# reunanen/annonet

Hardware: AMD Instinct MI355X
Metric: 227x227 RGB tiles/sec fwd+bwd @ batch 32 (higher is better)
Workload: dtype bf16; 1 GPU; training step (fwd+loss+bwd+SGD), batch 32x3x227x227 per GPU, encoder-decoder levels=2 width=1.0 K=3, random init; global_batch=32, parallelism=dp1

## Files before the change

annonet_amd/csrc/kernels_mfma.hip:

```cpp
#include <hip/hip_runtime.h>
#include <type_traits>

#include <algorithm>
#include <mutex>
#include <unordered_map>
#include <cstdio>
#include <vector>

#include "bnacc.h"
#include "common.h"
#include "kernels.h"

namespace anh {

void ensure_dynamic_lds(const void* kernel, size_t bytes) {
    if (bytes <= 64 * 1024) return;
    static std::mutex mu;
    static std::unordered_map<const void*, size_t> configured[64];
    int dev = 0;
    HIP_CHECK(hipGetDevice(&dev));
    std::lock_guard<std::mutex> lock(mu);
    size_t& have = configured[dev & 63][kernel];
    if (bytes > have) {
        HIP_CHECK(hipFuncSetAttribute(kernel, hipFuncAttributeMaxDynamicSharedMemorySize, (int)bytes));
// ... 845 lines not shown
        if constexpr (ONE_SET) {
            while (tile < total_tiles) {
                commit(ra, smem + (it & 1) * BUF_BYTES);
                if (tile + splits < total_tiles) fetch(ra, tile + splits);
                __syncthreads();
                tile += splits; ++it;
            }
        } else {
            if (tile + splits < total_tiles) fetch(rb, tile + splits);
            while (tile < total_tiles) {
                commit(ra, smem);
                if (tile + 2 * splits < total_tiles) fetch(ra, tile + 2 * splits);
                __syncthreads();
                tile += splits;
                if (tile >= total_tiles) break;
                commit(rb, smem + BUF_BYTES);
                if (tile + 2 * splits < total_tiles) fetch(rb, tile + 2 * splits);
                __syncthreads();
                tile += splits;
            }
        }
    } else {
        const int nt_mine = wave % NTC;
        int pofs[TPW][2], tofs[2];
#pragma unroll
        for (int i = 0; i < TPW; ++i) {
            const int j = wave + 4 * i, jc = j < 9 * NTC ? j : j - 4;
            const int tap = jc / NTC, ky = tap / 3, kx = tap - ky * 3;
            const int first = STRIDE == 1 ? ky * 34 + kx : (ky * 2 + (kx & 1)) * 33 + (kx >> 1);
            const int x_first = STRIDE == 1 ? kx : (kx >> 1);
#pragma unroll
            for (int rr = 0; rr < 2; ++rr) pofs[i][rr] = first * 64 + tr_lane_offset(lane, rr, x_first);
        }
#pragma unroll
        for (int rr = 0; rr < 2; ++rr) tofs[rr] = RECS * 64 + nt_mine * (TILE_PIX * 64) + tr_lane_offset(lane, rr, 0);
        f32x16 acc[TPW];
#pragma unroll
        for (int i = 0; i < TPW; ++i)
#pragma unroll
            for (int r = 0; r < 16; ++r) acc[i][r] = 0.f;
        for (; tile < total_tiles; tile += splits, ++it) {
            const char* lbuf = smem + (it & 1) * BUF_BYTES;
            const char* pa0[TPW];
            const char* pa1[TPW];
#pragma unroll
            for (int i = 0; i < TPW; ++i) { pa0[i] = lbuf + pofs[i][0]; pa1[i] = lbuf + pofs[i][1]; }
            const char* ta0 = lbuf + tofs[0];
            const char* ta1 = lbuf + tofs[1];
            __syncthreads();
            bf16x8 tf0, tf1, pf0[TPW], pf1[TPW];
            tf0 = tr_read8_at(ta0, ta1);
#pragma unroll
            for (int i = 0; i < TPW; ++i) pf0[i] = tr_read8_at(pa0[i], pa1[i]);
            wg_ksteps<0, KS, TPW, STRIDE, TRANS>(ta0, ta1, pa0, pa1, tf0, pf0, tf1, pf1, acc);
        }
        const size_t nw = (size_t)9 * a.c_in * a.c_out;
        float* out = a.partials + (size_t)split * nw;
        const int col = lane & 31, half = lane >> 5;
#pragma unroll
        for (int i = 0; i < TPW; ++i) {
            const int j = wave + 4 * i;
            if (j < 9 * NTC) {
                const int tap = j / NTC;
#pragma unroll
                for (int r = 0; r < 16; ++r) {
                    const int rowc = (r & 3) + 8 * (r >> 2) + 4 * half;
                    const int pch = cc + (TRANS ? col : rowc);
                    const int tch = tch0 + nt_mine * 32 + (TRANS ? rowc : col);
                    const int ci = TRANS ? tch : pch, co = TRANS ? pch : tch;
                    out[((size_t)tap * a.c_in + ci) * a.c_out + co] = acc[i][r];
                }
            }
        }
    }
}

__device__ __forceinline__ const char* swz_addr(const char* base, int rec, int key, int ks, int half) {
    return base + rec * 64 + ((((ks << 1) | half) ^ (key & 3)) << 4);
}
__device__ __forceinline__ bf16x8 lds_frag(const char* p) { return *reinterpret_cast<const bf16x8*>(p); }

struct GeoS1 {
    static constexpr int RECS = PATCH_PIX, ACC = 2;
    static constexpr bool RMW_PREFETCH = false;
    __device__ static void decode(int rec, int& py, int& px, int& key) { py = rec / PW; px = rec - py * PW; key = (px >> 2) & 3; }
    __device__ static int in_y0(int ty) { return ty * TH - 1; }
    __device__ static int in_x0(int tx) { return tx * TW - 1; }
    static constexpr int NB = 3;
    struct Bases { const char* x[3][2]; };
    __device__ static void init(Bases& b, const char* lds_x, int wave, int col, int half) {
#pragma unroll
        for (int kx = 0; kx < 3; ++kx)
#pragma unroll
            for (int ks = 0; ks < 2; ++ks) b.x[kx][ks] = swz_addr(lds_x, wave * 2 * PW + col + kx, (col + kx) >> 2, ks, half);
    }
    template <int NT>
    __device__ static void mfma(f32x16 (&acc)[ACC][NT], const Bases& b, const char* (&wb)[2]) {
        constexpr int C_OUT = NT * 32;
#pragma unroll
        for (int kx = 0; kx < 3; ++kx) {
#pragma unroll
            for (int ks = 0; ks < 2; ++ks) {
                bf16x8 xf[4];
#pragma unroll
                for (int r = 0; r < 4; ++r) xf[r] = lds_frag(b.x[kx][ks] + r * (PW * 64));
#pragma unroll
                for (int ky = 0; ky < 3; ++ky) {
                    const int tl = ky * 3 + kx;
#pragma unroll
                    for (int nt = 0; nt < NT; ++nt) {
                        const bf16x8 wf = lds_frag(wb[ks] + (tl * C_OUT + nt * 32) * 64);
#pragma unroll
                        for (int g = 0; g < 2; ++g) acc[g][nt] = __builtin_amdgcn_mfma_f32_32x32x16_bf16(wf, xf[g + ky], acc[g][nt], 0, 0, 0);
                    }
                }
            }
        }
    }
    __device__ static void load_filter_regs(bf16x8 (&wreg)[18], const char* (&wb)[2]) {
#pragma unroll
        for (int tl = 0; tl < 9; ++tl)
#pragma unroll
            for (int ks = 0; ks < 2; ++ks) wreg[tl * 2 + ks] = lds_frag(wb[ks] + (tl * 32) * 64);
    }
    __device__ static void mfma_wreg(f32x16 (&acc)[ACC][1], const Bases& b, const bf16x8 (&wreg)[18]) {
#pragma unroll
        for (int kx = 0; kx < 3; ++kx) {
#pragma unroll
            for (int ks = 0; ks < 2; ++ks) {
                bf16x8 xf[4];
#pragma unroll
                for (int r = 0; r < 4; ++r) xf[r] = lds_frag(b.x[kx][ks] + r * (PW * 64));
#pragma unroll
                for (int ky = 0; ky < 3; ++ky)
#pragma unroll
                    for (int g = 0; g < 2; ++g) acc[g][0] = __builtin_amdgcn_mfma_f32_32x32x16_bf16(wreg[(ky * 3 + kx) * 2 + ks], xf[g + ky], acc[g][0], 0, 0, 0);
            }
        }
    }
    __device__ static void out_pixel(int g, const ConvArgs& a, int n, int ty, int tx, int wave, int col, size_t& pix, bool& valid) {
        const int oy = ty * TH + wave * 2 + g, ox = tx * TW + col;
        valid = oy < a.h_out && ox < a.w_out;
        pix = ((size_t)n * a.h_out + (valid ? oy : 0)) * a.w_out + (valid ? ox : 0);
    }
};

struct GeoDown {
    static constexpr int RECS = 9 * 66, ACC = 1;
    static constexpr bool RMW_PREFETCH = false;
    __device__ static void decode(int rec, int& py, int& px, int& key) {
        py = rec / 66;
        const int rem = rec - py * 66, par = rem >= 33, u = rem - 33 * par;
        px = 2 * u + par; key = (u >> 2) & 3;
    }
    __device__ static int in_y0(int ty) { return ty * 8; }
    __device__ static int in_x0(int tx) { return tx * 64; }
    static constexpr int NB = 2;
    struct Bases { const char* x[2][2]; };
    __device__ static void init(Bases& b, const char* lds_x, int wave, int col, int half) {
#pragma unroll
        for (int kh = 0; kh < 2; ++kh)
#pragma unroll
            for (int ks = 0; ks < 2; ++ks) b.x[kh][ks] = swz_addr(lds_x, wave * 4 * 33 + col + kh, (col + kh) >> 2, ks, half);
    }
    template <int NT>
    __device__ static void mfma(f32x16 (&acc)[ACC][NT], const Bases& b, const char* (&wb)[2]) {
        constexpr int C_OUT = NT * 32;
#pragma unroll
        for (int tl = 0; tl < 9; ++tl) {
            const int ky = tl / 3, kx = tl - ky * 3;
#pragma unroll
            for (int ks = 0; ks < 2; ++ks) {
                const bf16x8 xf = lds_frag(b.x[kx >> 1][ks] + (ky * 2 + (kx & 1)) * (33 * 64));
#pragma unroll
                for (int nt = 0; nt < NT; ++nt) {
                    const bf16x8 wf = lds_frag(wb[ks] + (tl * C_OUT + nt * 32) * 64);
                    acc[0][nt] = __builtin_amdgcn_mfma_f32_32x32x16_bf16(wf, xf, acc[0][nt], 0, 0, 0);
                }
            }
        }
    }
    __device__ static void out_pixel(int, const ConvArgs& a, int n, int ty, int tx, int wave, int col, size_t& pix, bool& valid) {
        const int oy = ty * 4 + wave, ox = tx * 32 + col;
        valid = oy < a.h_out && ox < a.w_out;
        pix = ((size_t)n * a.h_out + (valid ? oy : 0)) * a.w_out + (valid ? ox : 0);
    }
};

struct GeoUp {
    static constexpr int RECS = 5 * 33, ACC = 4;
    static constexpr bool RMW_PREFETCH = true;
    __device__ static void decode(int rec, int& py, int& px, int& key) { py = rec / 33; px = rec - py * 33; key = (px >> 2) & 3; }
    __device__ static int in_y0(int ty) { return ty * 4 - 1; }
    __device__ static int in_x0(int tx) { return tx * 32 - 1; }
    static constexpr int NB = 2;
    struct Bases { const char* x[2][2]; };
    __device__ static void init(Bases& b, const char* lds_x, int wave, int col, int half) {
#pragma unroll
        for (int ib = 0; ib < 2; ++ib)
#pragma unroll
            for (int ks = 0; ks < 2; ++ks) b.x[ib][ks] = swz_addr(lds_x, wave * 33 + col + 1 - ib, (col + 1 - ib) >> 2, ks, half);
    }
    template <int NT>
    __device__ static void mfma(f32x16 (&acc)[ACC][NT], const Bases& b, const char* (&wb)[2]) {
        constexpr int C_OUT = NT * 32;
#pragma unroll
        for (int ks = 0; ks < 2; ++ks) {
            bf16x8 xf[2][2];
#pragma unroll
            for (int ia = 0; ia < 2; ++ia)
#pragma unroll
                for (int ib = 0; ib < 2; ++ib) xf[ia][ib] = lds_frag(b.x[ib][ks] + (1 - ia) * (33 * 64));
#pragma unroll
            for (int py = 0; py < 2; ++py)
#pragma unroll
                for (int px = 0; px < 2; ++px)
#pragma unroll
                    for (int ia = 0; ia < 2 - py; ++ia)
#pragma unroll
                        for (int ib = 0; ib < 2 - px; ++ib) {
                            const int tap = (py + 2 * ia) * 3 + px + 2 * ib;
#pragma unroll
                            for (int nt = 0; nt < NT; ++nt) {
                                const bf16x8 wf = lds_frag(wb[ks] + (tap * C_OUT + nt * 32) * 64);
                                acc[py * 2 + px][nt] = __builtin_amdgcn_mfma_f32_32x32x16_bf16(wf, xf[ia][ib], acc[py * 2 + px][nt], 0, 0, 0);
                            }
                        }
        }
    }
    __device__ static void out_pixel(int g, const ConvArgs& a, int n, int ty, int tx, int wave, int col, size_t& pix, bool& valid) {
        const int oy = 2 * (ty * 4 + wave) + (g >> 1), ox = 2 * (tx * 32 + col) + (g & 1);
        valid = oy < a.h_out && ox < a.w_out;
        pix = ((size_t)n * a.h_out + (valid ? oy : 0)) * a.w_out + (valid ? ox : 0);
    }
};

template <class G, int NT, int KIND, bool FWD = false, bool ACT = false, int PS = 0, bool HEAD = false>
__global__ __launch_bounds__(512, 2) void conv3x3_ws_kernel(ConvArgs a, int tiles_x, int tiles_y, int flip, long long* prof, int wres_, int e_off) {
#ifdef ANH_WS_PROFILE
    long long t_a = 0, t_b = 0, t_c = 0, t_d = 0, t0_;
    float prof_sink = 0.f;
    const bool prof_nostore = (wres_ >> 6) & 1;
    const long long t_entry = wall_clock64();
    long long t_loop = 0, t_loop_end = 0, c_loop = 0;
#define TICK() (t0_ = wall_clock64())
#define TOCK(acc_) (acc_ += wall_clock64() - t0_)
#else
#define TICK()
#define TOCK(acc_)
#endif
    static_assert(PS == 0 || PS == 1 || PS == 4 || PS == 5, "conv3x3_ws: producer-side forms 1 (sums), 4 (stores), 5 (both)");
    constexpr int NTHR = 512;
    constexpr int C_OUT = NT * 32, NP = (G::RECS * 4 + 255) / 256, W_ITEMS = 9 * C_OUT * 4, NW = (W_ITEMS + 255) / 256;
    constexpr int X_BYTES_ = G::RECS * 64, W_BYTES = 9 * C_OUT * 64, BUF = X_BYTES_ + W_BYTES;
    const int wres = wres_ & 1, bands = (wres_ >> 4) & 1;
    extern __shared__ __attribute__((aligned(16))) char smem[];
    const int n_slabs_l = a.c_red >> 5;
    const int x_stride = wres ? X_BYTES_ : BUF;
    const int w_base = 2 * X_BYTES_;
    const int tab_off = wres ? w_base + n_slabs_l * W_BYTES : 2 * BUF;
    float* tab = reinterpret_cast<float*>(smem + tab_off);

    const int hw_wave = __builtin_amdgcn_readfirstlane((int)threadIdx.x >> 6);
    const bool producer = hw_wave >= 4;
    const int wave = hw_wave & 3;
    const int lane = threadIdx.x & 63, tid = wave * 64 + lane, c16 = tid & 3;
    const int half = lane >> 5, col = lane & 31;
    const int co_base = blockIdx.y * C_OUT;
    const int H = a.h_in, W = a.w_in, c_red = a.c_red;
    const int n_slabs = c_red >> 5, n_tiles_all = tiles_x * tiles_y * a.n;
    const int band_len = (n_tiles_all + 7) >> 3;
    const int tile_first = bands ? (int)(blockIdx.x & 7) * band_len + (int)(blockIdx.x >> 3) : (int)blockIdx.x;
    const int gstep = bands ? (int)(gridDim.x >> 3) : (int)gridDim.x;
    const int n_tiles = bands ? min(n_tiles_all, ((int)(blockIdx.x & 7) + 1) * band_len) : n_tiles_all;
    constexpr bool CAN_STATS = G::ACC * NT <= 4 || FWD;
    const bool fuse_stats = !PS && !ACT && CAN_STATS && (a.stat_partials != nullptr || a.stat_acc != nullptr);
    const bool fuse_bnred = !FWD && (PS || CAN_STATS) && (a.bnred_partials != nullptr || a.bnred_acc != nullptr);
    constexpr bool PST = PS == 4 || PS == 5;
    const int stat_mode = fuse_stats ? 1 : (fuse_bnred && PS != 1 && PS != 5) ? 2 : 0;
    const bool ps = (PS == 1 || PS == 5) && fuse_bnred;
    const bool pst = PST && fuse_bnred;
    constexpr int E_BYTES = G::ACC * 128 * 64 * NT;
    constexpr int EK = 4 * NT, EQ_STEP = 256 / EK, ECH = G::ACC * 128 / EQ_STEP;
    float est[16];
    float* bnc = tab + c_red * 4;

    int tile = tile_first, slab = 0, it = 0;
    auto init_tables = [&]() __attribute__((always_inline)) {
        if (KIND == SRC_ACT || KIND == SRC_ACT2) {
            if (a.src.a_tab.acc) {
                const int sides = KIND == SRC_ACT2 ? 2 : 1;
                for (int i = threadIdx.x; i < sides * c_red; i += NTHR) {
                    const int side = i >= c_red, ch = i - side * c_red;
                    const BnTable& t = side ? a.src.b_tab : a.src.a_tab;
                    const BnFolded f = bnacc_fold_forward(t.acc, t.c, ch, t.pixels, t.gamma[ch], t.beta[ch], t.eps);
                    tab[2 * side * c_red + ch] = f.scale;
                    tab[(2 * side + 1) * c_red + ch] = f.shift;
                }
                if (KIND != SRC_ACT2) for (int i = threadIdx.x; i < c_red; i += NTHR) { tab[2 * c_red + i] = 0.f; tab[3 * c_red + i] = 0.f; }
            } else {
                for (int i = threadIdx.x; i < c_red; i += NTHR) {
                    tab[i] = a.src.a_scale[i];
                    tab[c_red + i] = a.src.a_shift[i];
                    tab[2 * c_red + i] = KIND == SRC_ACT2 ? a.src.b_scale[i] : 0.f;
                    tab[3 * c_red + i] = KIND == SRC_ACT2 ? a.src.b_shift[i] : 0.f;
                }
            }
        }
        if (ACT) {
            for (int i = threadIdx.x; i < C_OUT; i += NTHR) {
                bnc[i] = a.out_scale[co_base + i];
                bnc[C_OUT + i] = a.out_shift[co_base + i];
            }
        }
        if (fuse_bnred) {
            for (int i = threadIdx.x; i < C_OUT; i += NTHR) {
                bnc[i] = a.bnred_scale[co_base + i];
                bnc[C_OUT + i] = a.bnred_shift[co_base + i];
                bnc[2 * C_OUT + i] = a.bnred_mean[co_base + i];
                bnc[3 * C_OUT + i] = a.bnred_invstd[co_base + i];
            }
        }
        __syncthreads();
    };
    if (producer) {
        const bf16* wsrc = reinterpret_cast<const bf16*>(a.w_bf16);
        const bf16* xa = reinterpret_cast<const bf16*>(a.src.a);
        const bf16* xb = reinterpret_cast<const bf16*>(a.src.b);
        const size_t plane = (size_t)H * W * c_red;
        int pgeo[NP], pdst[NP];
    #pragma unroll
        for (int jj = 0; jj < NP; ++jj) {
            const int rec = min((tid >> 2) + 64 * jj, G::RECS - 1);
            int py, px, key;
            G::decode(rec, py, px, key);
            pgeo[jj] = py | (px << 8);
            pdst[jj] = rec * 64 + ((c16 ^ key) << 4);
        }
        int wsrc_off[NW], wdst[NW];
    #pragma unroll
        for (int j = 0; j < NW; ++j) {
            const int rec = min((tid >> 2) + 64 * j, 9 * C_OUT - 1);
            const int tl = rec / C_OUT, co = rec - tl * C_OUT;
            const int tap = flip ? 8 - tl : tl;
            wsrc_off[j] = (tap * a.c_out + co_base + co) * c_red + c16 * 8;
            wdst[j] = rec * 64 + ((c16 ^ ((co >> 2) & 3)) << 4);
        }
        u32x4 wraw[NW];
        struct Fetched {
            RawChunk<KIND> praw[NP];
            unsigned pok;
        };
        Fetched R0;
        const int per_img = tiles_x * tiles_y;
        const int step_x = gstep % tiles_x, step_y = (gstep / tiles_x) % tiles_y, step_n = gstep / per_img;
        int ftile = tile_first, fslab = 0;
        int ftx = ftile % tiles_x, fty = (ftile / tiles_x) % tiles_y, fn = ftile / per_img;
        constexpr bool NEED_MASK = KIND == SRC_ACT || KIND == SRC_ACT2;
        const int plane_bytes = (int)(unsigned)(plane * 2);
        int foff[NP];
        unsigned fpok = 0;
        auto enter_tile = [&]() __attribute__((always_inline)) {
            const int x0 = G::in_x0(ftx), y0 = G::in_y0(fty);
            fpok = 0;
    #pragma unroll
            for (int jj = 0; jj < NP; ++jj) {
                const int iy = y0 + (pgeo[jj] & 255), ix = x0 + (pgeo[jj] >> 8);
                const bool ok = (unsigned)iy < (unsigned)H && (unsigned)ix < (unsigned)W;
                foff[jj] = ok ? ((iy * W + ix) * c_red + c16 * 8) * 2 : (int)0xFFFFF000u;
                if constexpr (NEED_MASK) fpok |= (ok ? 1u : 0u) << jj;
            }
        };
        auto fetch = [&](Fetched& R) __attribute__((always_inline)) {
            const bf16* pa = xa + (size_t)fn * plane;
            const bf16* pb = (KIND == SRC_ACT2 || KIND == SRC_SUM2) ? xb + (size_t)fn * plane : nullptr;
            const int cc = fslab * 32;
            R.pok = fpok;
            const __amdgpu_buffer_rsrc_t ra = __builtin_amdgcn_make_buffer_rsrc(const_cast<bf16*>(pa), 0, plane_bytes, 0x00020000);
    #pragma unroll
            for (int jj = 0; jj < NP; ++jj) {
                const u32x4 v = __builtin_amdgcn_raw_buffer_load_b128(ra, foff[jj], cc * 2, 0);
                R.praw[jj].a = make_uint4(v[0], v[1], v[2], v[3]);
            }
            if constexpr (KIND == SRC_ACT2 || KIND == SRC_SUM2) {
                const __amdgpu_buffer_rsrc_t rb = __builtin_amdgcn_make_buffer_rsrc(const_cast<bf16*>(pb), 0, plane_bytes, 0x00020000);
    #pragma unroll
                for (int jj = 0; jj < NP; ++jj) {
                    const u32x4 v = __builtin_amdgcn_raw_buffer_load_b128(rb, foff[jj], cc * 2, 0);
                    R.praw[jj].b = make_uint4(v[0], v[1], v[2], v[3]);
                }
            }
            if (++fslab == n_slabs) {
                fslab = 0; ftile += gstep;
                ftx += step_x; if (ftx >= tiles_x) { ftx -= tiles_x; ++fty; }
                fty += step_y; if (fty >= tiles_y) { fty -= tiles_y; ++fn; }
                fn += step_n;
                if (ftile < n_tiles) enter_tile();
            }
        };
        const __amdgpu_buffer_rsrc_t rw = __builtin_amdgcn_make_buffer_rsrc(const_cast<bf16*>(wsrc), 0, 9 * a.c_out * c_red * 2, 0x00020000);
        auto fetch_w = [&](int slab_) __attribute__((always_inline)) {
    #pragma unroll
            for (int j = 0; j < NW; ++j) wraw[j] = __builtin_amdgcn_raw_buffer_load_b128(rw, wsrc_off[j] * 2, slab_ * 64, 0);
        };
        auto commit = [&](Fetched& R) __attribute__((always_inline)) {
            char* lbuf = smem + (it & 1) * x_stride;
            char* wbuf = lbuf + X_BYTES_;
            const bool stage_w = !wres && (it < 2 || n_slabs > 1);
            float sa[8], ta[8], sb[8], tb[8];
            if (KIND == SRC_ACT || KIND == SRC_ACT2) {
                const float* t0 = tab + slab * 32 + c16 * 8;
    #pragma unroll
                for (int j = 0; j < 8; ++j) {
                    sa[j] = t0[j]; ta[j] = t0[c_red + j];
                    sb[j] = KIND == SRC_ACT2 ? t0[2 * c_red + j] : 0.f;
                    tb[j] = KIND == SRC_ACT2 ? t0[3 * c_red + j] : 0.f;
                }
            }
    #pragma unroll
            for (int jj = 0; jj < NP; ++jj) {
                uint4 v = chunk_convert<KIND>(R.praw[jj], sa, ta, sb, tb);
                if constexpr (NEED_MASK) { if (!((R.pok >> jj) & 1u)) v = make_uint4(0u, 0u, 0u, 0u); }
                if ((tid >> 2) + 64 * jj < G::RECS) *reinterpret_cast<uint4*>(lbuf + pdst[jj]) = v;
            }
            if (stage_w) {
    #pragma unroll
                for (int j = 0; j < NW; ++j)
                    if ((tid >> 2) + 64 * j < 9 * C_OUT) *reinterpret_cast<u32x4*>(wbuf + wdst[j]) = wraw[j];
            }
        };
        if (ftile < n_tiles) { enter_tile(); fetch(R0); if (!wres) fetch_w(0); }
        if (wres && tile < n_tiles) {
            for (int sl = 0; sl < n_slabs; ++sl) {
                fetch_w(sl);
#pragma unroll
                for (int j = 0; j < NW; ++j)
                    if ((tid >> 2) + 64 * j < 9 * C_OUT) *reinterpret_cast<u32x4*>(smem + w_base + sl * W_BYTES + wdst[j]) = wraw[j];
            }
        }
        init_tables();
        float esc[8], esh[8];
        const int ek = tid & (EK - 1), eq0 = tid / EK;
        int hist1 = -1, hist2 = -1, hist1_it = 0, hist2_it = 0;
        if (PS == 1 || PS == 5) {
#pragma unroll
            for (int j = 0; j < 8; ++j) {
                esc[j] = bnc[ek * 8 + j]; esh[j] = bnc[C_OUT + ek * 8 + j];
                est[j] = 0.f; est[8 + j] = 0.f;
            }
        }
        const bf16* ylayer = reinterpret_cast<const bf16*>(a.bnred_y);
        unsigned epix[PST ? ECH : 1];
        auto estat_begin = [&](int et, u32x4 (&yv)[ECH], unsigned& evalid) __attribute__((always_inline)) {
            const int tx = et % tiles_x, ty = (et / tiles_x) % tiles_y, n = et / per_img;
            evalid = 0;
#pragma unroll
            for (int j = 0; j < ECH; ++j) {
                const int q = eq0 + EQ_STEP * j;
                size_t pix; bool valid;
                G::out_pixel(q >> 7, a, n, ty, tx, (q >> 5) & 3, q & 31, pix, valid);
                if (PS != 4) yv[j] = *reinterpret_cast<const u32x4*>(ylayer + pix * a.c_out + co_base + ek * 8);
                if constexpr (PST) epix[j] = (unsigned)pix;
                evalid |= (valid ? 1u : 0u) << j;
            }
        };
        auto estat_end = [&](int eit, const u32x4 (&yv)[ECH], unsigned evalid) __attribute__((always_inline)) {
            const char* eb = smem + e_off + (n_slabs == 1 ? (eit & 1) * E_BYTES : 0);
#pragma unroll
            for (int j = 0; j < ECH; ++j) {
                const int q = eq0 + EQ_STEP * j;
                const u32x4 dv = *reinterpret_cast<const u32x4*>(eb + q * (64 * NT) + ((ek ^ ebuf_swizzle<NT>(q)) << 4));
                if constexpr (PST) {
                    if ((evalid >> j) & 1u) store16(reinterpret_cast<bf16*>(a.out) + (size_t)epix[j] * a.c_out + co_base + ek * 8, make_uint4(dv[0], dv[1], dv[2], dv[3]));
                }
                if (PS != 4 && ((evalid >> j) & 1u)) {
#pragma unroll
                    for (int i = 0; i < 4; ++i)
#pragma unroll
                        for (int h2 = 0; h2 < 2; ++h2) {
                            const int c = 2 * i + h2;
                            const float d = h2 ? hi_f(dv[i]) : lo_f(dv[i]), y = h2 ? hi_f(yv[j][i]) : lo_f(yv[j][i]);
                            const float dz = fmaf(y, esc[c], esh[c]) > 0.f ? d : 0.f;
                            est[c] = fmaf(dz, y, est[c]);
                            est[8 + c] += dz;
                        }
                }
            }
        };
        auto one_item = [&](Fetched& R) __attribute__((always_inline)) {
            u32x4 eyv[PS ? ECH : 1];
            unsigned evalid = 0;
            const int et = hist2, eit = hist2_it;
            if constexpr (PS != 0) { if ((ps || pst) && et >= 0) estat_begin(et, eyv, evalid); }
            TICK();
            commit(R);
#ifdef ANH_WS_PROFILE
            __builtin_amdgcn_s_waitcnt(0xc07f);
#endif
            TOCK(t_a);
            TICK();
            if (ftile < n_tiles) fetch(R);
            if (!wres && n_slabs > 1 && (slab + 1 < n_slabs || tile + gstep < n_tiles)) fetch_w(slab + 1 < n_slabs ? slab + 1 : 0);
            if constexpr (PS != 0) { if ((ps || pst) && et >= 0) estat_end(eit, eyv, evalid); }
            TOCK(t_b);
            TICK();
            __syncthreads();
            TOCK(t_c);
            hist2 = hist1; hist2_it = hist1_it;
            hist1 = slab == n_slabs - 1 ? tile : -1; hist1_it = it;
            if (++slab == n_slabs) { slab = 0; tile += gstep; }
            ++it;
        };
#ifdef ANH_WS_PROFILE
        t_loop = wall_clock64();
        c_loop = clock64();
#endif
        while (tile < n_tiles) one_item(R0);
#ifdef ANH_WS_PROFILE
        t_loop_end = wall_clock64();
        c_loop = clock64() - c_loop;
#endif
        if constexpr (PS != 0) {
            if (ps || pst) {
                u32x4 eyv[ECH];
                unsigned evalid = 0;
                if (hist2 >= 0) { estat_begin(hist2, eyv, evalid); estat_end(hist2_it, eyv, evalid); }
                __syncthreads();
                if (hist1 >= 0) { estat_begin(hist1, eyv, evalid); estat_end(hist1_it, eyv, evalid); }
            }
        }
    } else {
        init_tables();
        typename G::Bases b0;
        G::init(b0, smem, wave, col, half);
        const char* wb0[2];
#pragma unroll
        for (int ks = 0; ks < 2; ++ks) wb0[ks] = swz_addr(smem, col, col >> 2, ks, half);
        f32x16 acc[G::ACC][NT];
        bf16x8 hw[2];
        float hbias[4] = {0.f, 0.f, 0.f, 0.f};
        if constexpr (HEAD) {
#pragma unroll
            for (int k = 0; k < 4; ++k) hbias[k] = k < a.head_k ? a.head_bias[k] : 0.f;
            head_operand(hw, a, col, half);
        }
        u32x4 old[FWD ? 1 : G::ACC][NT][2];
        u32x4 yraw[FWD ? 1 : G::ACC][NT][2];
        constexpr bool DEEP = !FWD && NT == 1 && G::RMW_PREFETCH;
        u32x4 old_n[DEEP ? G::ACC : 1][NT][2];
        const bool rmw_any = !FWD && G::RMW_PREFETCH && a.out_accumulate;
        const bool cons_bnred = fuse_bnred && PS != 1 && PS != 5;
        const bool pre_any = rmw_any || cons_bnred;
        auto prefetch_epilogue = [&](int t, auto& o, auto& y, bool want_old, bool want_y) __attribute__((always_inline)) {
            const int tx = t % tiles_x, ty = (t / tiles_x) % tiles_y, n = t / (tiles_x * tiles_y);
            const bf16* out = reinterpret_cast<const bf16*>(a.out);
            const bf16* yl = reinterpret_cast<const bf16*>(a.bnred_y);
#pragma unroll
            for (int g = 0; g < G::ACC; ++g) {
                size_t pix; bool valid;
                G::out_pixel(g, a, n, ty, tx, wave, col, pix, valid);
                const size_t e0 = pix * a.c_out + co_base + 8 * half;
#pragma unroll
                for (int nt = 0; nt < NT; ++nt)
#pragma unroll
                    for (int s2 = 0; s2 < 2; ++s2) {
                        if constexpr (!FWD) {
                            if (want_old) o[g][nt][s2] = *reinterpret_cast<const u32x4*>(out + e0 + nt * 32 + 16 * s2);
                            if (want_y) y[g][nt][s2] = *reinterpret_cast<const u32x4*>(yl + e0 + nt * 32 + 16 * s2);
                        }
                    }
            }
        };
        if (DEEP && pre_any && tile < n_tiles) prefetch_epilogue(tile, old, yraw, rmw_any, false);
        float stat[NT][2][16];
#pragma unroll
        for (int nt = 0; nt < NT; ++nt)
#pragma unroll
            for (int s2 = 0; s2 < 2; ++s2)
#pragma unroll
                for (int e = 0; e < 16; ++e) stat[nt][s2][e] = 0.f;
        constexpr bool WREG = std::is_same<G, GeoS1>::value && NT == 1;
        const bool wreg_on = WREG && n_slabs == 1 && !((wres_ >> 19) & 1);
        bf16x8 wreg[WREG ? 18 : 1];
        for (;;) {
            auto epilogue = [&](int et, int eit) __attribute__((always_inline)) {
                const int tx = et % tiles_x, ty = (et / tiles_x) % tiles_y, n = et / (tiles_x * tiles_y);
                const bool rmw = rmw_any;
#pragma unroll
                for (int g = 0; g < G::ACC; ++g) {
                    size_t pix; bool valid;
                    G::out_pixel(g, a, n, ty, tx, wave, col, pix, valid);
#ifdef ANH_WS_PROFILE
                    if (prof_nostore) valid = false;
#endif
                    if constexpr (HEAD) store_pixel_tiles_head(acc[g][0], a, pix, n, valid, half, bnc, C_OUT, hw, hbias);
                    else if constexpr (ACT) store_pixel_tiles_act<NT>(acc[g], a, pix, valid, half, co_base, bnc, C_OUT);
                    else {
                        const bool to_ebuf = ps || pst;
                        store_pixel_tiles_rmw<NT>(acc[g], a, pix, valid, half, co_base, old[FWD ? 0 : g], rmw, stat, stat_mode, yraw[FWD ? 0 : g], bnc,
                                                  to_ebuf ? smem + e_off + (n_slabs == 1 ? (eit & 1) * E_BYTES : 0) : nullptr, (g * 4 + wave) * 32 + col, !pst);
                    }
                }
                if constexpr (DEEP) {
                    if (pre_any) {
#pragma unroll
                        for (int g = 0; g < G::ACC; ++g)
#pragma unroll
                            for (int s2 = 0; s2 < 2; ++s2) old[g][0][s2] = old_n[g][0][s2];
                    }
                }
            };
            if (tile >= n_tiles) break;
            int ntile = tile, nslab = slab + 1;
            if (nslab == n_slabs) { nslab = 0; ntile += gstep; }
            const int boff = (it & 1) * x_stride;
            const int woff = wres ? w_base + slab * W_BYTES : boff + X_BYTES_;
            typename G::Bases b;
#pragma unroll
            for (int i = 0; i < G::NB; ++i)
#pragma unroll
                for (int ks = 0; ks < 2; ++ks) b.x[i][ks] = b0.x[i][ks] + boff;
            const char* wb[2] = {wb0[0] + woff, wb0[1] + woff};
            if (slab == 0) {
#pragma unroll
                for (int g = 0; g < G::ACC; ++g)
#pragma unroll
                    for (int nt = 0; nt < NT; ++nt)
#pragma unroll
                        for (int r = 0; r < 16; ++r) acc[g][nt][r] = 0.f;
            }
            TICK();
            __syncthreads();
            TOCK(t_c);
            TICK();
            const bool last_slab = slab == n_slabs - 1;
            if (pre_any && last_slab) {
                if constexpr (DEEP) {
                    if (tile + gstep < n_tiles) prefetch_epilogue(tile + gstep, old_n, yraw, rmw_any, false);
                    prefetch_epilogue(tile, old, yraw, false, cons_bnred);
                } else prefetch_epilogue(tile, old, yraw, rmw_any, cons_bnred);
            }
            if constexpr (WREG) {
                if (wreg_on) {
                    if (it == 0) G::load_filter_regs(wreg, wb);
                    G::mfma_wreg(acc, b, wreg);
                } else G::template mfma<NT>(acc, b, wb);
            } else G::template mfma<NT>(acc, b, wb);
#ifdef ANH_WS_PROFILE
            __builtin_amdgcn_sched_barrier(0);
#endif
            TOCK(t_a);
#ifdef ANH_WS_PROFILE
            TICK();
            if (last_slab) { asm volatile("v_mov_b32 %0, %1" : "=v"(prof_sink) : "v"(acc[0][0][0])); asm volatile("v_mov_b32 %0, %1" : "=v"(prof_sink) : "v"(acc[G::ACC - 1][NT - 1][15])); }
            __builtin_amdgcn_sched_barrier(0);
            TOCK(t_d);
#endif
            TICK();
            if (last_slab) epilogue(tile, it);
            TOCK(t_b);
            tile = ntile; slab = nslab; ++it;
        }
        if constexpr (PS != 0) { if (ps || pst) __syncthreads(); }
        if (stat_mode) {
            __syncthreads();
            float* red = reinterpret_cast<float*>(smem) + (size_t)(wave * 64 + lane) * (32 * NT);
#pragma unroll
            for (int nt = 0; nt < NT; ++nt)
#pragma unroll
// ... 27 lines not shown
            double* dst = fuse_stats ? a.stat_partials : a.bnred_partials;
            if (table) bnacc_add(table, (fuse_stats ? BNACC_SUM_Y : BNACC_SUM_DZ_XHAT) + which, a.c_out, co_base + ch, sum);
            else dst[((size_t)(co_base + ch) * 2 + which) * gridDim.x + blockIdx.x] = sum;
        }
    }
    if constexpr (PS == 1 || PS == 5) {
        if (ps) {
            __syncthreads();
            if (producer) {
                float* redw = reinterpret_cast<float*>(smem) + (size_t)tid * 16;
#pragma unroll
                for (int e = 0; e < 16; ++e) redw[e] = est[e];
            }
            __syncthreads();
            constexpr int GRP = 512 / (64 * NT);
            const int t = threadIdx.x / GRP, part = threadIdx.x % GRP;
            const int ch = t >> 1, which = t & 1, k = ch >> 3, j = ch & 7;
            const float* red = reinterpret_cast<const float*>(smem);
            double sum = 0.0;
#pragma unroll 4
            for (int m = part; m < EQ_STEP; m += GRP) sum += (double)red[(size_t)(k + EK * m) * 16 + which * 8 + j];
#pragma unroll
            for (int off = 1; off < GRP; off <<= 1) sum += __shfl_xor(sum, off, 64);
            {
                const double sum_dz = __shfl_down(sum, GRP, 64);
                if (which == 0) sum = (double)bnc[3 * C_OUT + ch] * (sum - (double)bnc[2 * C_OUT + ch] * sum_dz);
            }
            if (part == 0) {
                if (a.bnred_acc) bnacc_add(a.bnred_acc, BNACC_SUM_DZ_XHAT + which, a.c_out, co_base + ch, sum);
                else a.bnred_partials[((size_t)(co_base + ch) * 2 + which) * gridDim.x + blockIdx.x] = sum;
            }
        }
    }
    if (fuse_bnred && a.bnred_acc) bnacc_finish_backward(a.bnred_finish, (int)(gridDim.x * gridDim.y));
#ifdef ANH_WS_PROFILE
    if (prof && lane == 0) {
        long long* o = prof + ((size_t)(blockIdx.y * gridDim.x + blockIdx.x) * 8 + (producer ? 4 : 0) + wave) * 8;
        o[0] = t_a; o[1] = t_b; o[2] = t_c; o[3] = producer ? c_loop : it; o[4] = t_entry; o[5] = producer ? t_loop : t_d + (prof_sink == 12345.f ? 1 : 0); o[6] = t_loop_end; o[7] = wall_clock64();
    }
#endif
#undef TICK
#undef TOCK
}

int ws_target_wgs();

struct WsLayout { int wres; size_t lds; int ps ; int e_off; };
WsLayout ws_layout(const ConvArgs& a, int recs, int acc, int nt, bool with_bnred) {
    const size_t tables = (size_t)a.c_red * 16 + (size_t)nt * 32 * 16;
    const size_t x_bytes = (size_t)recs * 64, w_bytes = (size_t)9 * nt * 32 * 64;
    static const bool resident_on = !(getenv("ANH_WS_WEIGHT_RESIDENT") && atoi(getenv("ANH_WS_WEIGHT_RESIDENT")) == 0);
    const int n_slabs = a.c_red >> 5;
    const size_t resident_lds = 2 * x_bytes + (size_t)n_slabs * w_bytes + tables;
    WsLayout L{};
    L.wres = resident_on && n_slabs >= 2 && resident_lds <= 160 * 1024 && 2 * x_bytes + (size_t)n_slabs * w_bytes >= (size_t)32 * 1024 * nt;
    L.lds = L.wres ? resident_lds : 2 * (x_bytes + w_bytes) + tables;
    static const int ps_env = getenv("ANH_WS_PSTAT") ? atoi(getenv("ANH_WS_PSTAT")) : 7;
    int mode = 0;
    if (ps_env == 1) mode = acc == 4 ? 1 : 0;
    else if (ps_env == 8) mode = acc == 4 ? 1 : (acc * nt <= 4 ? 4 : 0);
    else mode = acc == 4 ? (nt == 1 ? 5 : 1) : (acc * nt <= 4 ? 4 : 0);
    const size_t e_total = (size_t)acc * 128 * 64 * nt * (n_slabs == 1 ? 2 : 1);
    if (mode && with_bnred && a.src.kind == SRC_RAW && !a.out_scale && !a.stat_partials && !a.stat_acc) {
        if (L.lds + e_total <= 160 * 1024) L.ps = mode;
        else if (n_slabs == 1 && resident_lds + e_total <= 160 * 1024 && resident_lds - tables >= 16 * 1024) { L.wres = 1; L.lds = resident_lds; L.ps = mode; }
    }
    L.e_off = L.ps ? (int)((L.lds + 15) / 16 * 16) : 0;
    if (L.ps) L.lds = (size_t)L.e_off + e_total;
    return L;
}

template <class G, int NT>
void launch_ws(const ConvArgs& a, int tiles_x, int tiles_y, int flip, hipStream_t s) {
    const int n_tiles = tiles_x * tiles_y * a.n, groups = a.c_out / (NT * 32);
    const dim3 grid((unsigned)std::max(1, std::min(n_tiles, ws_target_wgs() / groups)), (unsigned)groups);
    const WsLayout lay = ws_layout(a, G::RECS, G::ACC, NT, a.bnred_partials != nullptr || a.bnred_acc != nullptr);
    const int wres = lay.wres;
    const size_t lds = lay.lds;
    const int e_off = lay.e_off;
    static const int filter_regs_env = getenv("ANH_WS_FILTER_REGS") ? atoi(getenv("ANH_WS_FILTER_REGS")) : 1;
    const int ps = lay.ps;
    static const int bands_env = getenv("ANH_WS_XCD_BANDS") ? atoi(getenv("ANH_WS_XCD_BANDS")) : 1;
    const int bands = bands_env && grid.x % 8 == 0 && grid.x >= 8 ? 1 : 0;
    const int flags = wres | (bands << 4) | ((filter_regs_env ? 0 : 1) << 19);
    auto launch = [&](auto kernel) {
        const dim3 block(512);
        ensure_dynamic_lds(reinterpret_cast<const void*>(kernel), lds);
#ifndef ANH_WS_PROFILE
        hipLaunchKernelGGL(kernel, grid, block, lds, s, a, tiles_x, tiles_y, flip, (long long*)nullptr, flags, e_off);
#else
        static const int prof_on = getenv("ANH_WS_PROF") ? atoi(getenv("ANH_WS_PROF")) : 0;
        static long long* prof = nullptr;
        if (prof_on && !prof) HIP_CHECK(hipMalloc(&prof, 1024 * 12 * 8 * sizeof(long long)));
        static const int nostore = getenv("ANH_WS_PROF_NOSTORE") ? atoi(getenv("ANH_WS_PROF_NOSTORE")) : 0;
        hipLaunchKernelGGL(kernel, grid, block, lds, s, a, tiles_x, tiles_y, flip, prof_on ? prof : nullptr, flags | (nostore << 6), e_off);
        if (prof_on) {
            HIP_CHECK(hipStreamSynchronize(s));
            const int nwg = grid.x * grid.y, nw = 8, nc = 4;
            std::vector<long long> h((size_t)nwg * nw * 8);
            HIP_CHECK(hipMemcpy(h.data(), prof, h.size() * sizeof(long long), hipMemcpyDeviceToHost));
            double pa = 0, pb = 0, pc = 0, ca = 0, cb = 0, cc = 0, cd = 0, items = 0;
            long long first_entry = h[4], last_exit = h[7];
            double entry = 0, pro = 0, loop = 0, tail = 0, cycles = 0;
            for (int w = 0; w < nwg; ++w) {
                for (int v = 0; v < nw; ++v) { first_entry = std::min(first_entry, h[(w * nw + v) * 8 + 4]); last_exit = std::max(last_exit, h[(w * nw + v) * 8 + 7]); }
                for (int v = 0; v < nc; ++v) { ca += h[(w * nw + v) * 8]; cb += h[(w * nw + v) * 8 + 1]; cc += h[(w * nw + v) * 8 + 2]; cd += h[(w * nw + v) * 8 + 5]; }
                for (int v = nc; v < nw; ++v) { pa += h[(w * nw + v) * 8]; pb += h[(w * nw + v) * 8 + 1]; pc += h[(w * nw + v) * 8 + 2]; }
                items += h[(w * nw) * 8 + 3];
            }
            for (int w = 0; w < nwg; ++w)
                for (int v = nc; v < nw; ++v) {
                    const long long* o = &h[(w * nw + v) * 8];
                    entry += (double)(o[4] - first_entry); pro += (double)(o[5] - o[4]); loop += (double)(o[6] - o[5]); tail += (double)(o[7] - o[6]);
                    cycles += (double)o[3];
                }
            const double k = 1.0 / (4.0 * nwg) / 100.0;
            fprintf(stderr, "[ws prof] geo_recs=%d NT=%d kind=%d c_red=%d wgs=%d items/wg=%.1f | producer us: commit %.1f fetch %.1f barrier %.1f | consumer us: mfma %.1f drain %.1f store %.1f barrier %.1f"
                            " | kernel %.1f us = launch skew %.1f + prologue %.1f + loop %.1f + tail %.1f (+ drain to the last wave) | clock in the loop %.0f MHz\n",
                    G::RECS, NT, a.src.kind, a.c_red, nwg, items / nwg, pa * k, pb * k, pc * k, ca * k, cd * k, cb * k, cc * k,
                    (double)(last_exit - first_entry) / 100.0, entry * k, pro * k, loop * k, tail * k, loop > 0 ? cycles / loop * 100.0 : 0.0);
        }
#endif
    };
    if (a.out_scale) {
        ANH_REQUIRE(a.out_shift && !a.stat_partials && !a.bnred_partials && !a.stat_acc && !a.bnred_acc && !a.out_accumulate && !a.out2, "conv_ws: the activation-storing form takes no training epilogue");
        if (a.head_out) {
            if constexpr (std::is_same<G, GeoS1>::value && NT == 1) {
                ANH_REQUIRE(conv_head_in_epilogue_ok(a) && a.head_w && a.head_bias, "conv_ws: this layer cannot take the head in its epilogue");
                switch (a.src.kind) {
                    case SRC_RAW: launch(conv3x3_ws_kernel<G, NT, SRC_RAW, true, true, 0, true>); break;
                    case SRC_SUM2: launch(conv3x3_ws_kernel<G, NT, SRC_SUM2, true, true, 0, true>); break;
                    default: fail(ANH_ERR_INTERNAL, "conv_ws: the activation-storing form reads post-activation tensors");
                }
            } else fail(ANH_ERR_INTERNAL, "conv_ws: the head-in-epilogue form exists for the stride-1 32-channel kernel only");
            HIP_CHECK(hipGetLastError());
            return;
        }
        switch (a.src.kind) {
            case SRC_RAW: launch(conv3x3_ws_kernel<G, NT, SRC_RAW, true, true>); break;
            case SRC_SUM2: launch(conv3x3_ws_kernel<G, NT, SRC_SUM2, true, true>); break;
            default: fail(ANH_ERR_INTERNAL, "conv_ws: the activation-storing form reads post-activation tensors");
        }
        HIP_CHECK(hipGetLastError());
        return;
    }
    const bool fwd_form = (a.stat_partials || a.stat_acc) && !a.bnred_partials && !a.bnred_acc && !a.out_accumulate && !a.out2;
    if (fwd_form) {
        switch (a.src.kind) {
            case SRC_RAW: launch(conv3x3_ws_kernel<G, NT, SRC_RAW, true>); break;
            case SRC_ACT: launch(conv3x3_ws_kernel<G, NT, SRC_ACT, true>); break;
            case SRC_ACT2: launch(conv3x3_ws_kernel<G, NT, SRC_ACT2, true>); break;
            default: fail(ANH_ERR_INTERNAL, "conv_ws: no forward-only form for this source kind");
        }
        HIP_CHECK(hipGetLastError());
        return;
    }
    if (ps == 1) { launch(conv3x3_ws_kernel<G, NT, SRC_RAW, false, false, 1>); HIP_CHECK(hipGetLastError()); return; }
    if constexpr (G::ACC < 4 && G::ACC * NT <= 4) {
        if (ps == 4 && !a.out2) { launch(conv3x3_ws_kernel<G, NT, SRC_RAW, false, false, 4>); HIP_CHECK(hipGetLastError()); return; }
    }
    if (ps == 5 && !a.out2) { launch(conv3x3_ws_kernel<G, NT, SRC_RAW, false, false, 5>); HIP_CHECK(hipGetLastError()); return; }
    if (ps == 5) { launch(conv3x3_ws_kernel<G, NT, SRC_RAW, false, false, 1>); HIP_CHECK(hipGetLastError()); return; }
    switch (a.src.kind) {
        case SRC_RAW: launch(conv3x3_ws_kernel<G, NT, SRC_RAW>); break;
        case SRC_ACT: launch(conv3x3_ws_kernel<G, NT, SRC_ACT>); break;
        default: launch(conv3x3_ws_kernel<G, NT, SRC_ACT2>); break;
    }
    HIP_CHECK(hipGetLastError());
}

template <int CIN, bool BNBWD>
__global__ __launch_bounds__(256, 2) void wgrad_stem_mfma_kernel(WgradArgs a, WgSide dy_side, int tiles_x, int tiles_y, int total_tiles, int splits) {
    constexpr int ROWS = 25 * CIN, RT = (ROWS + 31) / 32, PLANE = 12 * 5 * 64 + 64;
    constexpr int IMG_THREADS = 12 * 4 * CIN;
    constexpr int BUF = 256 * 64 + (CIN + 1) * PLANE;
    extern __shared__ __attribute__((aligned(16))) char smem[];
    const int tid = threadIdx.x, lane = tid & 63, half = lane >> 5, col = lane & 31, c16 = tid & 3;
    const int wave = __builtin_amdgcn_readfirstlane(tid >> 6);

    for (int i = tid; i < PLANE / 4; i += 256) {
        reinterpret_cast<unsigned*>(smem + 256 * 64 + CIN * PLANE)[i] = 0u;
        reinterpret_cast<unsigned*>(smem + BUF + 256 * 64 + CIN * PLANE)[i] = 0u;
    }

    int a_off[RT];
#pragma unroll
    for (int rt = 0; rt < RT; ++rt) {
        const int r = rt * 32 + col;
        const int tap = r / CIN, ci = r - tap * CIN;
        const int ky = tap / 5, kx = tap - ky * 5;
        a_off[rt] = 256 * 64 + (r < ROWS ? ci * PLANE + (ky * 5 + kx) * 64 : CIN * PLANE) + half * 16 + wave * 2 * 320;
    }
    int g_off[2];
#pragma unroll
    for (int rr = 0; rr < 2; ++rr) g_off[rr] = wave * 2 * 32 * 64 + tr_lane_offset(lane, rr, 0);

    const bool img_thread = tid < IMG_THREADS;
    const int i_ci = tid % CIN, i_q = (tid / CIN) & 3, i_py = min(tid / (4 * CIN), 11);
    const int i_dst = 256 * 64 + i_ci * PLANE + i_py * 320 + i_q * 16;
    const int img_bytes = a.src.img_h * a.src.img_w * CIN;
    const int t_x = (tid >> 2) & 31, t_row0 = tid >> 7;
    const int gdst0 = (t_row0 * 32 + t_x) * 64 + ((c16 ^ ((t_x >> 2) & 3)) << 4);

    f32x16 acc[RT];
#pragma unroll
    for (int rt = 0; rt < RT; ++rt)
#pragma unroll
        for (int r = 0; r < 16; ++r) acc[rt][r] = 0.f;

    struct Regs {
        unsigned char ipx[12];
        unsigned gok;
        uint4 graw[4], yraw[4];
    };
    Regs R0;
    float bsc[8], bsf[8], bm[8], bis[8], bk0[8], bk1[8], bk2[8];
    if (BNBWD) {
#pragma unroll
        for (int j = 0; j < 8; ++j) {
            const int ch = c16 * 8 + j;
            bsc[j] = a.dy_scale[ch]; bsf[j] = a.dy_shift[ch]; bm[j] = a.dy_mean[ch]; bis[j] = a.dy_invstd[ch];
            bk0[j] = a.dy_coef[ch]; bk1[j] = a.dy_coef[32 + ch]; bk2[j] = a.dy_coef[64 + ch];
        }
    }
    const bf16* dyy = reinterpret_cast<const bf16*>(a.dy_y);
    const bf16* dyp = reinterpret_cast<const bf16*>(a.dy);
    const size_t dy_plane = (size_t)a.h_out * a.w_out * 32;
    struct TileAt { int x0, y0, n; };
    auto tile_at = [&](int tile) __attribute__((always_inline)) {
        const int tx = tile % tiles_x, ty = (tile / tiles_x) % tiles_y, n = tile / (tiles_x * tiles_y);
        return TileAt{tx * 32, ty * 8, n};
    };
    auto fetch_img = [&](Regs& R, const TileAt& t) __attribute__((always_inline)) {
        if (!img_thread) return;
        const __amdgpu_buffer_rsrc_t ri = __builtin_amdgcn_make_buffer_rsrc(const_cast<uint8_t*>(a.src.img + (size_t)t.n * a.src.img_sample_stride), 0, img_bytes, 0x00020000);
        const int iy = t.y0 - 2 + i_py, ix0 = t.x0 - 2 + 8 * i_q;
        const int top = a.src.win_top(t.n), left = a.src.win_left(t.n);
        const bool interior = iy >= 0 && iy < a.h_in && ix0 >= 0 && ix0 + 11 < a.w_in && top + iy >= 0 && top + iy < a.src.img_h && left + ix0 >= 0 && left + ix0 + 11 < a.src.img_w;
        if (interior) {
            const int off = ((top + iy) * a.src.img_w + left + ix0) * CIN + i_ci;
#pragma unroll
            for (int k = 0; k < 12; ++k) R.ipx[k] = __builtin_amdgcn_raw_buffer_load_b8(ri, off + k * CIN, 0, 0);
        } else {
            const int sy = min(max(top + iy, 0), a.src.img_h - 1);
#pragma unroll
            for (int k = 0; k < 12; ++k) {
                const int ix = ix0 + k, sx = min(max(left + ix, 0), a.src.img_w - 1);
                const bool ok = iy >= 0 && iy < a.h_in && ix >= 0 && ix < a.w_in;
                R.ipx[k] = __builtin_amdgcn_raw_buffer_load_b8(ri, ok ? (sy * a.src.img_w + sx) * CIN + i_ci : (int)0x7FFFFFF0, 0, 0);
            }
        }
// ... 662 lines not shown
```

Baseline: 20210 tiles/s.

## Walk stride-1 conv tiles in vertical strips and carry overlapping halo rows in LDS

Adds a strip-walk mode for the stride-1 weight-stationary 3x3 conv. Each workgroup now processes a contiguous run of tiles down a column instead of a grid-strided order. Between consecutive tiles in a strip, the bottom halo rows already staged in LDS are copied to the top of the next buffer, so the first staging pass skips its global loads. The mode is on by default through an env var and applies only when the reduction has at most two 32-channel slabs. It trades the XCD band interleaving and grid-stride load balance for contiguous runs, which can leave workgroups unevenly loaded.

```diff
diff --git a/annonet_amd/csrc/kernels_mfma.hip b/annonet_amd/csrc/kernels_mfma.hip
--- a/annonet_amd/csrc/kernels_mfma.hip
+++ b/annonet_amd/csrc/kernels_mfma.hip
@@ -951,6 +951,7 @@
 
 struct GeoS1 {
     static constexpr int RECS = PATCH_PIX, ACC = 2;
+    static constexpr int RL = PW, CARRY_ROWS = 2;
     static constexpr bool RMW_PREFETCH = false;
     __device__ static void decode(int rec, int& py, int& px, int& key) { py = rec / PW; px = rec - py * PW; key = (px >> 2) & 3; }
     __device__ static int in_y0(int ty) { return ty * TH - 1; }
@@ -1016,6 +1017,7 @@
 
 struct GeoDown {
     static constexpr int RECS = 9 * 66, ACC = 1;
+    static constexpr int RL = 66, CARRY_ROWS = 1;
     static constexpr bool RMW_PREFETCH = false;
     __device__ static void decode(int rec, int& py, int& px, int& key) {
         py = rec / 66;
@@ -1058,6 +1060,7 @@
 
 struct GeoUp {
     static constexpr int RECS = 5 * 33, ACC = 4;
+    static constexpr int RL = 33, CARRY_ROWS = 1;
     static constexpr bool RMW_PREFETCH = true;
     __device__ static void decode(int rec, int& py, int& px, int& key) { py = rec / 33; px = rec - py * 33; key = (px >> 2) & 3; }
     __device__ static int in_y0(int ty) { return ty * 4 - 1; }
@@ -1104,7 +1107,7 @@
     }
 };
 
-template <class G, int NT, int KIND, bool FWD = false, bool ACT = false, int PS = 0, bool HEAD = false>
+template <class G, int NT, int KIND, bool FWD = false, bool ACT = false, int PS = 0, bool HEAD = false, bool STRIPS = false>
 __global__ __launch_bounds__(512, 2) void conv3x3_ws_kernel(ConvArgs a, int tiles_x, int tiles_y, int flip, long long* prof, int wres_, int e_off) {
 #ifdef ANH_WS_PROFILE
     long long t_a = 0, t_b = 0, t_c = 0, t_d = 0, t0_;
@@ -1123,6 +1126,7 @@
     constexpr int C_OUT = NT * 32, NP = (G::RECS * 4 + 255) / 256, W_ITEMS = 9 * C_OUT * 4, NW = (W_ITEMS + 255) / 256;
     constexpr int X_BYTES_ = G::RECS * 64, W_BYTES = 9 * C_OUT * 64, BUF = X_BYTES_ + W_BYTES;
     const int wres = wres_ & 1, bands = (wres_ >> 4) & 1;
+    constexpr bool strips = STRIPS;
     extern __shared__ __attribute__((aligned(16))) char smem[];
     const int n_slabs_l = a.c_red >> 5;
     const int x_stride = wres ? X_BYTES_ : BUF;
@@ -1139,9 +1143,21 @@
     const int H = a.h_in, W = a.w_in, c_red = a.c_red;
     const int n_slabs = c_red >> 5, n_tiles_all = tiles_x * tiles_y * a.n;
     const int band_len = (n_tiles_all + 7) >> 3;
-    const int tile_first = bands ? (int)(blockIdx.x & 7) * band_len + (int)(blockIdx.x >> 3) : (int)blockIdx.x;
-    const int gstep = bands ? (int)(gridDim.x >> 3) : (int)gridDim.x;
-    const int n_tiles = bands ? min(n_tiles_all, ((int)(blockIdx.x & 7) + 1) * band_len) : n_tiles_all;
+    const int run_len = (n_tiles_all + (int)gridDim.x - 1) / (int)gridDim.x;
+    const int run = (gridDim.x & 7) == 0 ? (int)(blockIdx.x & 7) * (int)(gridDim.x >> 3) + (int)(blockIdx.x >> 3) : (int)blockIdx.x;
+    const int tile_first = strips ? run * run_len : bands ? (int)(blockIdx.x & 7) * band_len + (int)(blockIdx.x >> 3) : (int)blockIdx.x;
+    const int gstep = strips ? 1 : bands ? (int)(gridDim.x >> 3) : (int)gridDim.x;
+    const int n_tiles = strips ? min(n_tiles_all, (run + 1) * run_len)
+                               : bands ? min(n_tiles_all, ((int)(blockIdx.x & 7) + 1) * band_len) : n_tiles_all;
+    auto tile_decode = [&](int t, int& tx, int& ty, int& n) __attribute__((always_inline)) {
+        n = t / (tiles_x * tiles_y);
+        if (strips) { ty = t % tiles_y; tx = (t / tiles_y) % tiles_x; }
+        else { tx = t % tiles_x; ty = (t / tiles_x) % tiles_y; }
+    };
+    constexpr int CR = G::CARRY_ROWS * G::RL, SRC0 = G::RECS - CR;
+    constexpr bool CARRY = STRIPS && CR >= 64;
+    static_assert(!STRIPS || CR >= 64, "conv3x3_ws: a strip walk without a staging pass to skip");
+    static_assert(!CARRY || (SRC0 % G::RL == 0 && SRC0 / 64 + 1 < NP), "conv3x3_ws: the carried records keep their column (swizzle key) and are owned by two staging passes");
     constexpr bool CAN_STATS = G::ACC * NT <= 4 || FWD;
     const bool fuse_stats = !PS && !ACT && CAN_STATS && (a.stat_partials != nullptr || a.stat_acc != nullptr);
     const bool fuse_bnred = !FWD && (PS || CAN_STATS) && (a.bnred_partials != nullptr || a.bnred_acc != nullptr);
@@ -1219,12 +1235,15 @@
         struct Fetched {
             RawChunk<KIND> praw[NP];
             unsigned pok;
+            bool carry;
         };
         Fetched R0;
         const int per_img = tiles_x * tiles_y;
         const int step_x = gstep % tiles_x, step_y = (gstep / tiles_x) % tiles_y, step_n = gstep / per_img;
         int ftile = tile_first, fslab = 0;
-        int ftx = ftile % tiles_x, fty = (ftile / tiles_x) % tiles_y, fn = ftile / per_img;
+        int ftx, fty, fn;
+        tile_decode(ftile, ftx, fty, fn);
+        bool fcarry = false;
         constexpr bool NEED_MASK = KIND == SRC_ACT || KIND == SRC_ACT2;
         const int plane_bytes = (int)(unsigned)(plane * 2);
         int foff[NP];
@@ -1234,6 +1253,7 @@
             fpok = 0;
     #pragma unroll
             for (int jj = 0; jj < NP; ++jj) {
+                if (CARRY && jj == 0 && fcarry) continue;
                 const int iy = y0 + (pgeo[jj] & 255), ix = x0 + (pgeo[jj] >> 8);
                 const bool ok = (unsigned)iy < (unsigned)H && (unsigned)ix < (unsigned)W;
                 foff[jj] = ok ? ((iy * W + ix) * c_red + c16 * 8) * 2 : (int)0xFFFFF000u;
@@ -1245,9 +1265,11 @@
             const bf16* pb = (KIND == SRC_ACT2 || KIND == SRC_SUM2) ? xb + (size_t)fn * plane : nullptr;
             const int cc = fslab * 32;
             R.pok = fpok;
+            R.carry = fcarry;
             const __amdgpu_buffer_rsrc_t ra = __builtin_amdgcn_make_buffer_rsrc(const_cast<bf16*>(pa), 0, plane_bytes, 0x00020000);
     #pragma unroll
             for (int jj = 0; jj < NP; ++jj) {
+                if (CARRY && jj == 0 && fcarry) continue;
                 const u32x4 v = __builtin_amdgcn_raw_buffer_load_b128(ra, foff[jj], cc * 2, 0);
                 R.praw[jj].a = make_uint4(v[0], v[1], v[2], v[3]);
             }
@@ -1255,15 +1277,21 @@
                 const __amdgpu_buffer_rsrc_t rb = __builtin_amdgcn_make_buffer_rsrc(const_cast<bf16*>(pb), 0, plane_bytes, 0x00020000);
     #pragma unroll
                 for (int jj = 0; jj < NP; ++jj) {
+                    if (CARRY && jj == 0 && fcarry) continue;
                     const u32x4 v = __builtin_amdgcn_raw_buffer_load_b128(rb, foff[jj], cc * 2, 0);
                     R.praw[jj].b = make_uint4(v[0], v[1], v[2], v[3]);
                 }
             }
             if (++fslab == n_slabs) {
                 fslab = 0; ftile += gstep;
-                ftx += step_x; if (ftx >= tiles_x) { ftx -= tiles_x; ++fty; }
-                fty += step_y; if (fty >= tiles_y) { fty -= tiles_y; ++fn; }
-                fn += step_n;
+                if (strips) {
+                    if (++fty == tiles_y) { fty = 0; if (++ftx == tiles_x) { ftx = 0; ++fn; } }
+                    fcarry = CARRY && fty != 0;
+                } else {
+                    ftx += step_x; if (ftx >= tiles_x) { ftx -= tiles_x; ++fty; }
+                    fty += step_y; if (fty >= tiles_y) { fty -= tiles_y; ++fn; }
+                    fn += step_n;
+                }
                 if (ftile < n_tiles) enter_tile();
             }
         };
@@ -1286,11 +1314,25 @@
                     tb[j] = KIND == SRC_ACT2 ? t0[3 * c_red + j] : 0.f;
                 }
             }
+            u32x4 cv = {0u, 0u, 0u, 0u};
+            int cofs = 0;
+            const bool carry = CARRY && R.carry;
+            if constexpr (CARRY) {
+                if (carry) {
+                    cofs = (tid >> 2) >= SRC0 % 64 ? pdst[SRC0 / 64] : pdst[SRC0 / 64 + 1];
+                    const char* sbuf = n_slabs == 1 ? smem + ((it & 1) ^ 1) * x_stride : lbuf;
+                    cv = *reinterpret_cast<const u32x4*>(sbuf + cofs);
+                }
+            }
     #pragma unroll
             for (int jj = 0; jj < NP; ++jj) {
+                if (CARRY && jj == 0 && carry) continue;
                 uint4 v = chunk_convert<KIND>(R.praw[jj], sa, ta, sb, tb);
                 if constexpr (NEED_MASK) { if (!((R.pok >> jj) & 1u)) v = make_uint4(0u, 0u, 0u, 0u); }
                 if ((tid >> 2) + 64 * jj < G::RECS) *reinterpret_cast<uint4*>(lbuf + pdst[jj]) = v;
+            }
+            if constexpr (CARRY) {
+                if (carry) *reinterpret_cast<u32x4*>(lbuf + cofs - SRC0 * 64) = cv;
             }
             if (stage_w) {
     #pragma unroll
@@ -1321,7 +1363,8 @@
         const bf16* ylayer = reinterpret_cast<const bf16*>(a.bnred_y);
         unsigned epix[PST ? ECH : 1];
         auto estat_begin = [&](int et, u32x4 (&yv)[ECH], unsigned& evalid) __attribute__((always_inline)) {
-            const int tx = et % tiles_x, ty = (et / tiles_x) % tiles_y, n = et / per_img;
+            int tx, ty, n;
+            tile_decode(et, tx, ty, n);
             evalid = 0;
 #pragma unroll
             for (int j = 0; j < ECH; ++j) {
@@ -1421,7 +1464,8 @@
         const bool cons_bnred = fuse_bnred && PS != 1 && PS != 5;
         const bool pre_any = rmw_any || cons_bnred;
         auto prefetch_epilogue = [&](int t, auto& o, auto& y, bool want_old, bool want_y) __attribute__((always_inline)) {
-            const int tx = t % tiles_x, ty = (t / tiles_x) % tiles_y, n = t / (tiles_x * tiles_y);
+            int tx, ty, n;
+            tile_decode(t, tx, ty, n);
             const bf16* out = reinterpret_cast<const bf16*>(a.out);
             const bf16* yl = reinterpret_cast<const bf16*>(a.bnred_y);
 #pragma unroll
@@ -1453,7 +1497,8 @@
         bf16x8 wreg[WREG ? 18 : 1];
         for (;;) {
             auto epilogue = [&](int et, int eit) __attribute__((always_inline)) {
-                const int tx = et % tiles_x, ty = (et / tiles_x) % tiles_y, n = et / (tiles_x * tiles_y);
+                int tx, ty, n;
+                tile_decode(et, tx, ty, n);
                 const bool rmw = rmw_any;
 #pragma unroll
                 for (int g = 0; g < G::ACC; ++g) {
@@ -1647,7 +1692,15 @@
     const int ps = lay.ps;
     static const int bands_env = getenv("ANH_WS_XCD_BANDS") ? atoi(getenv("ANH_WS_XCD_BANDS")) : 1;
     const int bands = bands_env && grid.x % 8 == 0 && grid.x >= 8 ? 1 : 0;
+    static const int carry_env = getenv("ANH_WS_ROW_CARRY") ? atoi(getenv("ANH_WS_ROW_CARRY")) : 1;
+    constexpr bool CAN_STRIP = std::is_same<G, GeoS1>::value;
+    const bool strips = CAN_STRIP && (carry_env & 1) && (a.c_red >> 5) <= 2;
     const int flags = wres | (bands << 4) | ((filter_regs_env ? 0 : 1) << 19);
+#define ANH_WS_LAUNCH(...)                                                                            \
+    do {                                                                                              \
+        if constexpr (CAN_STRIP) { if (strips) { launch(conv3x3_ws_kernel<__VA_ARGS__, false, true>); break; } }  \
+        launch(conv3x3_ws_kernel<__VA_ARGS__>);                                                       \
+    } while (0)
     auto launch = [&](auto kernel) {
         const dim3 block(512);
         ensure_dynamic_lds(reinterpret_cast<const void*>(kernel), lds);
@@ -1712,26 +1765,27 @@
     const bool fwd_form = (a.stat_partials || a.stat_acc) && !a.bnred_partials && !a.bnred_acc && !a.out_accumulate && !a.out2;
     if (fwd_form) {
         switch (a.src.kind) {
-            case SRC_RAW: launch(conv3x3_ws_kernel<G, NT, SRC_RAW, true>); break;
-            case SRC_ACT: launch(conv3x3_ws_kernel<G, NT, SRC_ACT, true>); break;
-            case SRC_ACT2: launch(conv3x3_ws_kernel<G, NT, SRC_ACT2, true>); break;
+            case SRC_RAW: ANH_WS_LAUNCH(G, NT, SRC_RAW, true, false, 0); break;
+            case SRC_ACT: ANH_WS_LAUNCH(G, NT, SRC_ACT, true, false, 0); break;
+            case SRC_ACT2: ANH_WS_LAUNCH(G, NT, SRC_ACT2, true, false, 0); break;
             default: fail(ANH_ERR_INTERNAL, "conv_ws: no forward-only form for this source kind");
         }
         HIP_CHECK(hipGetLastError());
         return;
     }
-    if (ps == 1) { launch(conv3x3_ws_kernel<G, NT, SRC_RAW, false, false, 1>); HIP_CHECK(hipGetLastError()); return; }
+    if (ps == 1) { ANH_WS_LAUNCH(G, NT, SRC_RAW, false, false, 1); HIP_CHECK(hipGetLastError()); return; }
     if constexpr (G::ACC < 4 && G::ACC * NT <= 4) {
-        if (ps == 4 && !a.out2) { launch(conv3x3_ws_kernel<G, NT, SRC_RAW, false, false, 4>); HIP_CHECK(hipGetLastError()); return; }
-    }
-    if (ps == 5 && !a.out2) { launch(conv3x3_ws_kernel<G, NT, SRC_RAW, false, false, 5>); HIP_CHECK(hipGetLastError()); return; }
-    if (ps == 5) { launch(conv3x3_ws_kernel<G, NT, SRC_RAW, false, false, 1>); HIP_CHECK(hipGetLastError()); return; }
+        if (ps == 4 && !a.out2) { ANH_WS_LAUNCH(G, NT, SRC_RAW, false, false, 4); HIP_CHECK(hipGetLastError()); return; }
+    }
+    if (ps == 5 && !a.out2) { ANH_WS_LAUNCH(G, NT, SRC_RAW, false, false, 5); HIP_CHECK(hipGetLastError()); return; }
+    if (ps == 5) { ANH_WS_LAUNCH(G, NT, SRC_RAW, false, false, 1); HIP_CHECK(hipGetLastError()); return; }
     switch (a.src.kind) {
-        case SRC_RAW: launch(conv3x3_ws_kernel<G, NT, SRC_RAW>); break;
-        case SRC_ACT: launch(conv3x3_ws_kernel<G, NT, SRC_ACT>); break;
-        default: launch(conv3x3_ws_kernel<G, NT, SRC_ACT2>); break;
+        case SRC_RAW: ANH_WS_LAUNCH(G, NT, SRC_RAW, false, false, 0); break;
+        case SRC_ACT: ANH_WS_LAUNCH(G, NT, SRC_ACT, false, false, 0); break;
+        default: ANH_WS_LAUNCH(G, NT, SRC_ACT2, false, false, 0); break;
     }
     HIP_CHECK(hipGetLastError());
+#undef ANH_WS_LAUNCH
 }
 
 template <int CIN, bool BNBWD>
```

New measurement: 20010 tiles/s. No clear change (-1.0%).
